# facebookresearch/habitat-lab

Hardware: AMD Instinct MI355X
Metric: env-steps/sec (SPS) PointNav RGB-D 256x256, 64 envs x 128 rollout (higher is better)
Workload: dtype f32; 1 GPU; PointNav SimpleCNN+GRU, 64 envs x 128 steps, 256x256 RGB-D synthetic; envs_per_gpu=64, rollout_steps=128, ppo_epoch=4, num_mini_batch=4, parallelism=dp1

## Files before the change

habitat-lab_amd/csrc/gemm_ops.hip:

```cpp
#include "igemm.h"
#include "igemm_dma.h"
#include "igemm_dma_wgrad.h"
#include "igemm_bf3.h"
#include "igemm_bf3_ws.h"
#include "dense_bf3.h"
#include "obs_conv_bf3.h"
#include "obs_conv_bf3_ws.h"
#include "obs_conv_patch.h"
#include "wgrad3x3_bf3.h"
#include "conv2_fwd_strip.h"
#include "conv2_dgrad_strip.h"
#include "conv3_dgrad_strip.h"
#include "obs_wgrad_bf3.h"
#include "obs_wgrad_strip.h"
#include "conv_patch_bf3.h"
#include "wgrad3x3_patch.h"
#include "prob_build.h"
#include <stdlib.h>

#include <atomic>

#include "../../include/habitat_amd.h"

namespace hab {
// ... 141 lines not shown
    if (form == HAB_CONV_DGRAD_FORM_CONV3_STRIP) HAB_TRY_FORM(conv3_dgrad_strip(d, dy, wd, mask, add, dx, stream));
    if (d.stride > 1) {
        ConvDgradMergedProb q;
        HAB_TRY(check_conv(d));
        q.g = make_geom(d);
        if (ConvDgradMergedProb::applicable(q.g)) {
            q.dy = dy; q.w = wd; q.mask = mask; q.add = add; q.dx = dx;
            q.finish();
            if (matrix_path_on(MP_RC) && q.M > 64)
                return by_width<false>(q.M, q.N, [&](auto t) { return bf3_launch<ConvDgradMergedProb, decltype(t)>(q, ws, ws_floats, 256, stream); });
            if (q.dma_ok()) return dma_launch<false>(q, ws, ws_floats, 1024, stream);
        }
    }
    for (int ph = 0; ph < d.stride; ++ph)
        for (int pw = 0; pw < d.stride; ++pw) {
            ConvDgradProb p;
            HAB_TRY(build(p, d, dy, wd, mask, add, dx, ph, pw));
            if (p.Hc <= 0 || p.Wc <= 0) continue;
            if (patch3x3_wanted(d, p.M) && p.K > 0) {
                const int rc = conv_patch_bf3_dispatch(p, patch3x3_geom(dy, p.g.Ho, p.g.Wo, d.Cout, d.H, d.W, d.pad - 2, 1), ws, ws_floats, stream);
                if (rc == HAB_OK) continue;
                if (rc != HAB_NOT_APPLICABLE) return rc;
            }
            if (p.K <= 0) {
                p.M = d.B * p.Hc * p.Wc;
                dgrad_empty_class_kernel<<<1024, 256, 0, stream>>>(p);
                HAB_LAUNCH_CHECK();
                continue;
            }
            HAB_TRY(run_igemm(p, ws, ws_floats, stream));
        }
    return HAB_OK;
}
int conv_wgrad(const ConvDesc& d, const float* x, const float* dy, float* dw_oihw, float* dbias, float* ws, size_t ws_floats,
               hipStream_t stream) {
    ConvWgradProb p;
    HAB_TRY(build(p, d, x, dy, dw_oihw, dbias));
    if (ws && matrix_path_on(MP_WGRAD_STRIP | MP_IJ_WGRAD) && wgrad3x3_bf3_shape(p))
        HAB_TRY_FORM(wgrad3x3_bf3(p, ws, ws_floats, stream));
    if (ws && !matrix_path_on(MP_IJ_WGRAD)) {
        ConvWgradProb q = p;
        q.colsum = nullptr;
        auto bias_grad = [&] { return dbias ? colsum(dy, p.N, p.K, p.N, dbias, 0, ws, ws_floats, stream) : HAB_OK; };
        if (wgrad3x3_patch_ok(p)) {
            HAB_TRY(bias_grad());
            return wgrad3x3_patch(q, ws, ws_floats, stream);
        }
        if (d.pad == 0 && p.N <= 32 && wgrad_dma_ok(q)) {
            HAB_TRY(bias_grad());
            if (rows_fit(q.M, 288, 256)) return igemm_dma_wgrad_launch<3, 3, 1>(q, ws, ws_floats, 1024, stream);
            return igemm_dma_wgrad_launch<2, 4, 1>(q, ws, ws_floats, 1024, stream);
        }
    }
    return run_igemm(p, ws, ws_floats, stream);
}
static int choose_obs_wgrad(const ObsConvWgradProb& p, const float* ws, size_t ws_floats) {
    if (!(matrix_path_on(MP_OBS) && p.quad && p.K > 4096)) return HAB_OBS_WGRAD_FORM_IGEMM;
    if (matrix_path_on(MP_OBS_PATCH | MP_OBS) && obs_wgrad_strip_covers(p, ws, ws_floats)) return HAB_OBS_WGRAD_FORM_STRIP;
    return obs_wgrad_bf3_covers(p, ws, ws_floats) ? HAB_OBS_WGRAD_FORM_IM2COL : HAB_OBS_WGRAD_FORM_IGEMM;
}
int obs_conv_wgrad(const ConvDesc& d, const ObsView& obs, const float* dy, float* dw_oihw, float* dbias, float* ws,
                   size_t ws_floats, hipStream_t stream) {
    ObsConvWgradProb p;
    HAB_TRY(build(p, d, obs, dy, dw_oihw, dbias));
    const int form = choose_obs_wgrad(p, ws, ws_floats);
    if (form == HAB_OBS_WGRAD_FORM_STRIP) HAB_TRY_FORM(obs_wgrad_strip_launch(p, ws, ws_floats, stream));
    if (form >= HAB_OBS_WGRAD_FORM_IM2COL) HAB_TRY_FORM(obs_wgrad_bf3_launch(p, ws, ws_floats, stream));
    return run_igemm(p, ws, ws_floats, stream);
}

static bool dense_wanted(long long M, long long N, long long K) {
    if (!matrix_path_on(MP_DENSE | MP_RC)) return false;
// ... 221 lines not shown
    return obs_conv_fwd(mk(B, H, W, o.C, Cout, KH, KW, stride, pad), o, w_fwd, bias, y, relu, ws, ws_floats, stream);
}
extern "C" int hab_obs_conv2d_fwd_form(const uint8_t* rgb, const float* depth, const int* rows, const float* w_fwd,
                                       const float* bias, float* y, int B, int H, int W, int Cout, int KH, int KW, int stride,
                                       int pad, int relu, const float* ws, size_t ws_floats) {
    if ((!rgb && !depth) || !w_fwd || !y) return HAB_ERR_ARG;
    ObsView o = mkobs(rgb, depth, rows, H, W);
    ObsConvFwdProb p;
    const int r = build(p, mk(B, H, W, o.C, Cout, KH, KW, stride, pad), o, w_fwd, bias, y, relu);
    if (r != HAB_OK) return r;
    return choose_obs_fwd(p, ws, ws_floats, nullptr);
}
extern "C" int hab_conv2d_dgrad(const float* dy, const float* w_dgrad, const float* relu_mask, const float* add, float* dx,
                                int B, int H, int W, int C, int Cout, int KH, int KW, int stride, int pad, float* ws,
                                size_t ws_floats, hipStream_t stream) {
    if (!dy || !w_dgrad || !dx) return HAB_ERR_ARG;
    return conv_dgrad(mk(B, H, W, C, Cout, KH, KW, stride, pad), dy, w_dgrad, relu_mask, add, dx, ws, ws_floats, stream);
}
extern "C" int hab_conv2d_dgrad_form(const float* dy, const float* w_dgrad, const float* relu_mask, const float* add, float* dx,
                                     int B, int H, int W, int C, int Cout, int KH, int KW, int stride, int pad, const float* ws,
                                     size_t ws_floats) {
    (void)ws; (void)ws_floats;
    if (!dy || !w_dgrad || !dx) return HAB_ERR_ARG;
    const ConvDesc d = mk(B, H, W, C, Cout, KH, KW, stride, pad);
    const int r = check_conv(d);
    if (r != HAB_OK) return r;
    return choose_conv_dgrad(d, dy, w_dgrad, relu_mask, add, dx);
}
extern "C" int hab_conv2d_wgrad(const float* x, const float* dy, float* dw_oihw, float* dbias, int B, int H, int W, int C, int Cout,
                                int KH, int KW, int stride, int pad, float* ws, size_t ws_floats, hipStream_t stream) {
    if (!x || !dy || !dw_oihw) return HAB_ERR_ARG;
    return conv_wgrad(mk(B, H, W, C, Cout, KH, KW, stride, pad), x, dy, dw_oihw, dbias, ws, ws_floats, stream);
}
extern "C" int hab_obs_conv2d_wgrad(const uint8_t* rgb, const float* depth, const int* rows, const float* dy, float* dw_oihw,
                                    float* dbias, int B, int H, int W, int Cout, int KH, int KW, int stride, int pad, float* ws,
                                    size_t ws_floats, hipStream_t stream) {
    if ((!rgb && !depth) || !dy || !dw_oihw) return HAB_ERR_ARG;
    ObsView o = mkobs(rgb, depth, rows, H, W);
    return obs_conv_wgrad(mk(B, H, W, o.C, Cout, KH, KW, stride, pad), o, dy, dw_oihw, dbias, ws, ws_floats, stream);
}
extern "C" int hab_obs_conv2d_wgrad_form(const uint8_t* rgb, const float* depth, const int* rows, const float* dy, float* dw_oihw,
                                         float* dbias, int B, int H, int W, int Cout, int KH, int KW, int stride, int pad, const float* ws,
                                         size_t ws_floats) {
    if ((!rgb && !depth) || !dy || !dw_oihw) return HAB_ERR_ARG;
    ObsView o = mkobs(rgb, depth, rows, H, W);
    ObsConvWgradProb p;
    const int r = build(p, mk(B, H, W, o.C, Cout, KH, KW, stride, pad), o, dy, dw_oihw, dbias);
    if (r != HAB_OK) return r;
    return choose_obs_wgrad(p, ws, ws_floats);
}
extern "C" int hab_linear_fwd(const float* x, int ldx, const float* w, int ldw, const float* bias, float* y, int ldy, int M,
                              int N, int K, int relu, int accumulate, float* ws, size_t ws_floats, hipStream_t stream) {
    return linear_fwd(x, ldx, w, ldw, bias, y, ldy, M, N, K, relu, accumulate, ws, ws_floats, stream);
}
extern "C" int hab_linear_dgrad(const float* dy, int lddy, const float* w, int ldw, const float* relu_mask, int ldmask,
                                float* dx, int lddx, int M, int n_in, int n_out, int accumulate, float* ws, size_t ws_floats,
                                hipStream_t stream) {
    return linear_dgrad(dy, lddy, w, ldw, relu_mask, ldmask, n_in, dx, lddx, M, n_in, n_out, accumulate, ws, ws_floats, stream);
}
extern "C" int hab_linear_wgrad(const float* dy, int lddy, const float* x, int ldx, float* dw, int lddw, int M, int n_out,
                                int n_in, int perm_c, int perm_hw, int accumulate, float* ws, size_t ws_floats,
                                hipStream_t stream) {
    return linear_wgrad(dy, lddy, x, ldx, dw, lddw, M, n_out, n_in, perm_c, perm_hw, accumulate, ws, ws_floats, stream);
}
extern "C" int hab_debug_dense_trace(long long* out320) {
    return (int)hipMemcpyFromSymbol(out320, HIP_SYMBOL(hab::dn_trace), sizeof(long long) * 8 * 8 * 5);
// ... 16 lines not shown
```

habitat-lab_amd/csrc/ops.h:

```cpp
#pragma once
#include "hab_common.h"

namespace hab {

struct ConvDesc {
    int B, H, W, C, Cout, KH, KW, stride, pad;
    int Creal = 0;
    int Ho() const { return (H + 2 * pad - KH) / stride + 1; }
    int Wo() const { return (W + 2 * pad - KW) / stride + 1; }
};
struct ObsView;

int conv_fwd(const ConvDesc& d, const float* x, const float* wf, const float* bias, float* y, int relu, float* ws,
             size_t ws_floats, hipStream_t stream);
int obs_conv_fwd(const ConvDesc& d, const ObsView& obs, const float* wf, const float* bias, float* y, int relu, float* ws,
                 size_t ws_floats, hipStream_t stream, const void* wimg = nullptr);
int64_t obs_conv_weight_image_floats();
int obs_conv_weight_image(const float* wf, int Cout, int KH, int KW, int C, void* img, hipStream_t stream);
int conv_dgrad(const ConvDesc& d, const float* dy, const float* wd, const float* mask, const float* add, float* dx,
               float* ws, size_t ws_floats, hipStream_t stream);
int conv_wgrad(const ConvDesc& d, const float* x, const float* dy, float* dw_oihw, float* dbias, float* ws, size_t ws_floats,
               hipStream_t stream);
int obs_conv_wgrad(const ConvDesc& d, const ObsView& obs, const float* dy, float* dw_oihw, float* dbias, float* ws,
                   size_t ws_floats, hipStream_t stream);
// ... 43 lines not shown
                  const int* frag_env, const int* frag_start, int F, int H, float* hinit, hipStream_t stream,
                  const int* env_first = nullptr);
int rnn_seq_layer_forward(int rnn_type, int H, const RnnLayerParams& lp, const RnnWork& wk, const float* x, int ldx,
                          const float* hinit, const float* cinit, const PackInfo& pk, float* ws, size_t ws_floats,
                          hipStream_t stream);
int rnn_seq_wave_forward(int rnn_type, int H, int L, const RnnLayerParams* lp, const RnnWork* wk, const float* x, int ldx,
                         const float* const* hinit, const float* const* cinit, const PackInfo& pk, float* ws, size_t ws_floats,
                         hipStream_t stream);
int rnn_seq_wave_backward(int rnn_type, int H, int L, const RnnLayerParams* lp, const float* const* w_ih_t, const RnnWork* wk, const float* x0,
                          int ldx0, const float* dout, float* dx0, int lddx0, const float* dx_mask, int ldmask, int mask_cols,
                          const PackInfo& pk, float* scratch , float* ws, size_t ws_floats, hipStream_t stream);
int rnn_step_layer_forward(int rnn_type, int H, const RnnLayerParams& lp, const float* x, int ldx, const float* h_in, int h_in_stride,
                           const float* c_in, int c_in_stride, const uint8_t* masks, int n, float* gi_scratch, float* h_out,
                           int h_out_stride, float* c_out, int c_out_stride, float* ws, size_t ws_floats, hipStream_t stream);
int rnn_seq_layer_backward(int rnn_type, int H, const RnnLayerParams& lp, const RnnWork& wk, const float* x, int ldx,
                           const float* dout, float* dx, int lddx, const float* dx_mask, int ldmask, int mask_cols,
                           const PackInfo& pk, float* scratch , float* ws, size_t ws_floats,
                           hipStream_t stream);
enum MatrixPath : int {
    MP_RC = 1 << 0,
    MP_OBS = 1 << 1,
    MP_IJ = 1 << 2,
    MP_IJ_WGRAD = 1 << 3,
    MP_PATCH3X3 = 1 << 4,
    MP_WS = 1 << 5,
    MP_OBS_PATCH = 1 << 6,
    MP_WGRAD_STRIP = 1 << 7,
    MP_CONV2_FWD = 1 << 8,
    MP_CONV2_DGRAD = 1 << 9,
    MP_DENSE = 1 << 10,
    MP_DENSE_ALL = 1 << 11,
    MP_RNN_STEPWISE = 1 << 12,
    MP_OBS_PATCH_PLAIN = 1 << 13,
    MP_DEFAULT = 2047,
};
int matrix_path_bits();
inline bool matrix_path_on(int bits) { return (matrix_path_bits() & bits) == bits; }
int rnn_tm_prepare(const uint8_t* masks, const int* rows, int B, uint8_t* frame_mask, int* iota, hipStream_t stream);
int rnn_tm_layer_forward(int rnn_type, int H, const RnnLayerParams& lp, const RnnWork& wk, const float* x, int ldx, const float* hinit,
                         const float* cinit, const uint8_t* frame_mask, int n, int T_total, int t0, int t1, float* ws, size_t ws_floats,
                         hipStream_t stream);
int rnn_tm_layer_backward(int rnn_type, int H, const RnnLayerParams& lp, const RnnWork& wk, const float* dout, float* dx, int lddx,
                          const float* dx_mask, int ldmask, int mask_cols, const uint8_t* frame_mask, const int* iota, int n, int T, int t0,
                          int t1, float* scratch, float* ws, size_t ws_floats, hipStream_t stream);
int rnn_tm_layer_param_grads(int rnn_type, int H, const RnnLayerParams& lp, const RnnWork& wk, const float* x, int ldx, int P, float* ws,
                             size_t ws_floats, hipStream_t stream);

}
```

habitat-lab_amd/csrc/wgrad3x3_bf3.h:

```cpp
#pragma once
#include "igemm_bf3.h"

namespace hab {

struct W3bArgs {
    const float* x;
    const float* dy;
    float* partial;
    int B, H, Ho;
    int strips;
    int items;
    int sign_schedule;
    int colsum;
};

template <int C32, int N32, int W, int PAD, int KHW, int S, int R, int KS, int NS>
struct W3bCfg {
    static constexpr int C = 32 * C32, N = 32 * N32, WP = W + 2 * PAD, Wo = (WP - KHW) / S + 1, NT = 64 * KHW * KS * NS, NW = N32 / NS;
    static constexpr int XRS = (R - 1) * S + KHW;
    static constexpr int XROWS = XRS * WP, NPIX = R * Wo, NQ = (NPIX + 3) / 4, NSTEPS = (NQ + 3) / 4, YROWS = NSTEPS * 16;
    static constexpr int XU = XRS * W * C / 4, YU = R * Wo * N / 4, XPT = (XU + NT - 1) / NT, YPT = (YU + NT - 1) / NT;
    static constexpr int X_HALF = XROWS * 32, Y_HALF = YROWS * 32;
    static constexpr size_t LDS_BYTES = (size_t)(3 * C32 * X_HALF + 3 * N32 * Y_HALF) * 2;
    static constexpr int WH = (WP + 1) / 2;
    __host__ __device__ static constexpr int xcol(int w) { return S == 2 ? (w & 1) * WH + (w >> 1) : w; }
    __host__ __device__ static constexpr int tap_col(int kw) { return S == 2 ? (kw & 1) * WH + (kw >> 1) : kw; }
    static_assert(S == 1 || S == 2, "");
    static_assert(LDS_BYTES % 16 == 0 && N32 % NS == 0 && NT % (N / 4) == 0 && LDS_BYTES >= (size_t)NT * 16, "");
};

typedef short w3b_v4s __attribute__((ext_vector_type(4)));
typedef short w3b_v8s __attribute__((ext_vector_type(8)));

__device__ __forceinline__ w3b_v4s w3b_tr_read(const unsigned short* p) {
    return __builtin_amdgcn_ds_read_tr16_b64_v4i16((__attribute__((address_space(3))) w3b_v4s*)p);
}
__device__ __forceinline__ bf16x8 w3b_join(const w3b_v4s lo, const w3b_v4s hi) {
    return __builtin_bit_cast(bf16x8, __builtin_shufflevector(lo, hi, 0, 1, 2, 3, 4, 5, 6, 7));
}

template <int C32, int N32, int W, int PAD, int KHW, int S, int R, int KS, int NS>
__global__ void __launch_bounds__(64 * KHW * KS * NS) wgrad3x3_bf3_kernel(const W3bArgs a) {
    using Cfg = W3bCfg<C32, N32, W, PAD, KHW, S, R, KS, NS>;
    constexpr int C = Cfg::C, N = Cfg::N, WP = Cfg::WP, Wo = Cfg::Wo, NT = Cfg::NT, NW = Cfg::NW;
    extern __shared__ __attribute__((aligned(16))) unsigned short smem16[];
    unsigned short* xs = smem16;
    unsigned short* ys = smem16 + 3 * C32 * Cfg::X_HALF;
    const int t = threadIdx.x, lane = t & 63;
    const int wave = __builtin_amdgcn_readfirstlane(t >> 6);
    const int kh = wave % KHW, ns = (wave / KHW) % NS, ks = wave / (KHW * NS);

    for (int i = t; i < (int)(Cfg::LDS_BYTES / 16); i += NT) reinterpret_cast<u32x4*>(smem16)[i] = u32x4{0u, 0u, 0u, 0u};

    const int xcd = blockIdx.x & 7, jw = blockIdx.x >> 3, wg_per_xcd = gridDim.x >> 3;
    const int per_xcd = (a.items + 7) >> 3, per_wg = (per_xcd + wg_per_xcd - 1) / wg_per_xcd;
    const int xcd_end = min(a.items, (xcd + 1) * per_xcd);
    const int first = min(xcd_end, xcd * per_xcd + jw * per_wg), last = min(xcd_end, first + per_wg);

    const bool flip = a.sign_schedule && (blockIdx.x & 1);
    const unsigned sgn2 = flip ? 0x80008000u : 0u;

// ... 109 lines not shown
        __syncthreads();
    }

    const int li = lane & 31, hi = lane >> 5;
    constexpr int MROWS = KHW * KHW * C;
    const size_t slab = (size_t)(MROWS + (a.colsum ? 1 : 0)) * N;
    float* out = a.partial + (size_t)(blockIdx.x * KS + ks) * slab;
#pragma unroll
    for (int kw = 0; kw < KHW; ++kw)
#pragma unroll
        for (int hc = 0; hc < C32; ++hc)
#pragma unroll
            for (int hn = 0; hn < NW; ++hn)
#pragma unroll
                for (int v = 0; v < 16; ++v) {
                    const int ci = (v & 3) + 8 * (v >> 2) + 4 * hi;
                    const float val = acc[kw][hc][hn][v];
                    out[(size_t)((kh * KHW + kw) * C + hc * 32 + ci) * N + (ns * NW + hn) * 32 + li] = flip ? -val : val;
                }
    if (a.colsum) {
        float* red = reinterpret_cast<float*>(smem16);
        *reinterpret_cast<f32x4*>(red + t * 4) = cs;
        __syncthreads();
        if (t < N) {
            float sum = 0.f;
            for (int q = (t >> 2); q < NT; q += N / 4) sum += red[q * 4 + (t & 3)];
            a.partial[(size_t)(blockIdx.x * KS) * slab + (size_t)MROWS * N + t] = sum;
#pragma unroll
            for (int z = 1; z < KS; ++z) a.partial[(size_t)(blockIdx.x * KS + z) * slab + (size_t)MROWS * N + t] = 0.f;
        }
    }
}

template <int C32, int N32, int W, int PAD, int KHW, int S, int R, int KS, int NS>
inline int wgrad3x3_bf3_run(const ConvWgradProb& p, float* ws, size_t ws_floats, hipStream_t stream) {
    using Cfg = W3bCfg<C32, N32, W, PAD, KHW, S, R, KS, NS>;
    const ConvGeom& g = p.g;
    W3bArgs a;
    a.x = p.x; a.dy = p.dy; a.partial = ws; a.B = g.B; a.H = g.H; a.Ho = g.Ho;
    a.strips = g.Ho / R;
    a.items = g.B * a.strips;
    a.sign_schedule = bf3_sign_schedule();
    a.colsum = p.colsum != nullptr;
    auto kern = wgrad3x3_bf3_kernel<C32, N32, W, PAD, KHW, S, R, KS, NS>;
    static const hipError_t attr_err = (Cfg::LDS_BYTES > 64 * 1024) ? hipFuncSetAttribute(reinterpret_cast<const void*>(kern), hipFuncAttributeMaxDynamicSharedMemorySize, (int)Cfg::LDS_BYTES) : hipSuccess;
    if (attr_err != hipSuccess) return (int)attr_err;
    const size_t MN = (size_t)(KHW * KHW * Cfg::C + (a.colsum ? 1 : 0)) * Cfg::N;
    const int per_cu = (int)std::min<size_t>(Cfg::NT <= 192 ? 4 : 2, (160 * 1024) / Cfg::LDS_BYTES);
    int grid = 256 * std::max(per_cu, 1);
    while (grid > 8 && (grid > a.items || (size_t)grid * KS * MN > ws_floats)) grid -= 8;
    if ((size_t)grid * KS * MN > ws_floats || (grid < 128 && a.items >= 1024)) return 1;
    kern<<<grid, Cfg::NT, Cfg::LDS_BYTES, stream>>>(a);
    HAB_LAUNCH_CHECK();
    igemm_splitk_reduce<ConvWgradProb>(p, ws, grid * KS, stream);
    HAB_LAUNCH_CHECK();
    return HAB_OK;
}

inline int wgrad3x3_bf3_shape(const ConvWgradProb& p) {
    const ConvGeom& g = p.g;
    if (p.Creal != g.C || (size_t)g.B * g.H * g.W * std::max(g.C, g.Cout) >= 0x7fffffffull / 2) return 0;
    if (g.KH == 4 && g.KW == 4 && g.stride == 2 && g.C == 32 && g.Cout == 64 && g.W == 63 && g.pad == 0 && g.Ho % 2 == 0) return 4;
    if (!(g.KH == 3 && g.KW == 3 && g.stride == 1)) return 0;
    if (g.C == 64 && g.Cout == 32 && g.W == 30 && g.pad == 0 && g.Ho % 2 == 0) return 1;
    if (g.C == 32 && g.Cout == 32 && g.W == 32 && g.pad == 1 && g.Ho % 4 == 0) return 2;
    if (g.C == 64 && g.Cout == 64 && g.W == 16 && g.pad == 1 && g.Ho % 4 == 0) return 3;
    return 0;
}
inline int wgrad3x3_bf3(const ConvWgradProb& p, float* ws, size_t ws_floats, hipStream_t stream) {
    if (!ws) return HAB_ERR_ARG;
    switch (wgrad3x3_bf3_shape(p)) {
        case 1: return wgrad3x3_bf3_run<2, 1, 30, 0, 3, 1, 2, 2, 1>(p, ws, ws_floats, stream);
        case 2: return wgrad3x3_bf3_run<1, 1, 32, 1, 3, 1, 2, 1, 1>(p, ws, ws_floats, stream);
        case 3: return wgrad3x3_bf3_run<2, 2, 16, 1, 3, 1, 4, 1, 2>(p, ws, ws_floats, stream);
        case 4: return wgrad3x3_bf3_run<1, 2, 63, 0, 4, 2, 2, 2, 1>(p, ws, ws_floats, stream);
    }
    return HAB_ERR_UNSUPPORTED;
}

}
```

habitat-lab_amd/habitat_amd/_lib.py:

```python
from __future__ import annotations

import ctypes as C
import os
from ctypes import POINTER, c_char_p, c_double, c_float, c_int, c_int32, c_int64, c_size_t, c_uint8, c_uint32, c_void_p

_HERE = os.path.dirname(os.path.abspath(__file__))
LIB_PATH = os.path.join(_HERE, "libhabitat_amd.so")

vp = c_void_p
ALLREDUCE_FN = C.CFUNCTYPE(None, c_void_p, c_int, c_float, c_void_p)
GRAD_READY_FN = C.CFUNCTYPE(None, c_int64, c_int64, c_void_p)


class HabError(RuntimeError):
    pass


class PolicyDesc(C.Structure):
    _fields_ = [(n, c_int32) for n in (
        "arch", "backbone", "baseplanes", "normalize_visual_inputs", "rnn_type", "rnn_layers", "hidden", "num_actions",
        "H", "W", "has_rgb", "has_depth", "goal_dim", "max_frames", "max_envs", "visual_order", "has_semantic",
        "num_object_categories", "has_compass", "has_gps", "action_dist", "gauss_flags")] + [("gauss_min_std", c_float),
                                                                                                ("gauss_max_std", c_float),
                                                                                                ("pointgoal_dim", c_int32),
# ... 51 lines not shown
    "hab_nav2d_rearr_vel_step": (c_int, [vp] * 15 + [c_uint32, c_uint32] + [c_int] * 9 + [c_float, c_int, c_int, vp]),
    "hab_nav2d_rearr_geo_bytes": (c_int, []),
    "hab_nav2d_rearr_geo_build": (c_int, [vp, c_size_t, vp, vp, c_int, c_int, c_int, c_int, vp]),
    "hab_nav2d_rearr_step_geo": (c_int, [vp] * 16 + [c_uint32, c_uint32] + [c_int] * 8 + [vp]),
    "hab_nav2d_rearr_vel_step_geo": (c_int, [vp] * 16 + [c_uint32, c_uint32] + [c_int] * 9 + [c_float, c_int, c_int, vp]),
    "hab_nav2d_rearr_oracle": (c_int, [vp, c_size_t] + [vp] * 6 + [c_int] * 3 + [vp]),
    "hab_nav2d_social_state_bytes": (c_int, []),
    "hab_nav2d_social_step": (c_int, [vp] * 14 + [c_uint32, c_uint32] + [c_int] * 8 + [c_float, c_int, c_float, c_int, c_int, vp]),
    "hab_obs_resize_crop": (c_int, [vp, vp, c_int, c_int, c_int, c_int, c_int, c_int, c_int, c_int, c_int, c_int, c_int, c_int, vp]),
    "hab_obs_resize_crop_form": (c_int, [vp, c_int, c_int, c_int, c_int, c_int, c_int, c_int, c_int]),
    "hab_obs_project": (c_int, [vp, c_int, vp, c_int, c_int, c_int, c_int, c_int, vp, vp, c_int, c_int, vp]),
    "hab_rollout_step_stats": (c_int, [vp, vp, vp, vp, vp, vp, vp, c_int, c_int, vp]),
    "hab_compute_returns": (c_int, [vp, vp, vp, vp, vp, c_int, c_int, c_float, c_float, c_int, c_int, vp]),
    "hab_advantages": (c_int, [vp, vp, vp, c_int, c_int, vp, vp, vp]),
    "hab_ppo_loss": (c_int, [vp, vp, vp, vp, vp, vp, vp, vp, c_int, c_float, c_float, c_float, c_int, vp, vp, vp, vp, vp]),
    "hab_ppo_loss_ver": (c_int, [vp, vp, vp, vp, vp, vp, vp, vp, c_int, c_float, c_float, c_float, c_int, vp, vp, vp, c_int64, vp, c_float,
                                 vp, vp, vp, vp, vp]),
    "hab_dagger_mix": (c_int, [vp, vp, vp, vp, vp, vp, c_float, c_float, vp, vp, vp, c_int, vp]),
    "hab_bc_loss": (c_int, [vp, vp, vp, vp, vp, vp, c_int, c_float, c_float, vp, vp, vp, vp, vp]),
    "hab_lagrange_adam_step": (c_int, [vp, vp, vp, vp, c_float, c_float, c_float, c_float, c_float, c_int, c_float, c_float, vp, vp]),
    "hab_ver_compute_returns": (c_int, [vp, vp, vp, vp, vp, vp, vp, vp, c_int, c_double, c_double, vp]),
    "hab_ver_is_coeffs": (c_int, [vp, c_int, c_int, c_int, vp, vp, vp]),
    "hab_clip_adam_step": (c_int, [vp, vp, vp, vp, c_size_t, vp, c_int, c_float, c_float, c_float, c_float, c_float,
                                   c_float, c_int, vp, vp]),
    "hab_sample_actions": (c_int, [vp, vp, vp, c_int, c_int, c_int, vp]),
    "hab_set_matrix_path": (c_int, [c_int]),
    "hab_conv2d_fwd": (c_int, [vp, vp, vp, vp] + [c_int] * 10 + [vp, c_size_t, vp]),
    "hab_obs_conv2d_fwd": (c_int, [vp, vp, vp, vp, vp, vp] + [c_int] * 9 + [vp, c_size_t, vp]),
    "hab_conv2d_dgrad": (c_int, [vp, vp, vp, vp, vp] + [c_int] * 9 + [vp, c_size_t, vp]),
    "hab_conv2d_wgrad": (c_int, [vp, vp, vp, vp] + [c_int] * 9 + [vp, c_size_t, vp]),
    "hab_obs_conv2d_wgrad": (c_int, [vp, vp, vp, vp, vp, vp] + [c_int] * 8 + [vp, c_size_t, vp]),
    "hab_obs_conv2d_wgrad_form": (c_int, [vp, vp, vp, vp, vp, vp] + [c_int] * 8 + [vp, c_size_t]),
    "hab_conv2d_dgrad_form": (c_int, [vp, vp, vp, vp, vp] + [c_int] * 9 + [vp, c_size_t]),
    "hab_obs_conv2d_fwd_form": (c_int, [vp, vp, vp, vp, vp, vp] + [c_int] * 9 + [vp, c_size_t]),
    "hab_linear_fwd": (c_int, [vp, c_int, vp, c_int, vp, vp, c_int, c_int, c_int, c_int, c_int, c_int, vp, c_size_t, vp]),
    "hab_linear_dgrad": (c_int, [vp, c_int, vp, c_int, vp, c_int, vp, c_int, c_int, c_int, c_int, c_int, vp, c_size_t, vp]),
    "hab_linear_wgrad": (c_int, [vp, c_int, vp, c_int, vp, c_int, c_int, c_int, c_int, c_int, c_int, c_int, vp, c_size_t, vp]),
    "hab_colsum": (c_int, [vp, c_int, c_int, c_int, vp, c_int, vp, c_size_t, vp]),
    "hab_repack_conv_weight": (c_int, [vp, vp, vp, c_int, c_int, c_int, c_int, c_int, vp]),
    "hab_repack_flatten_weight": (c_int, [vp, vp, c_int, c_int, c_int, vp]),
    "hab_transpose2d": (c_int, [vp, vp, c_int, c_int, vp]),
    "hab_obs_ingest_pool": (c_int, [vp, vp, vp, vp, vp, c_int, c_int, c_int, c_int, c_int, c_int, c_int, vp]),
    "hab_obs_ingest_pool_sensors": (c_int, [vp, vp, vp, vp, c_int, vp, vp, c_int, c_int, c_int, c_int, vp, vp, vp, vp, vp, vp]),
    "hab_fused_gather": (c_int, [vp, vp, c_int, vp, vp, c_int, c_int, c_int, c_int, c_int, vp]),
    "hab_channel_moments": (c_int, [vp, c_int64, c_int, c_int, vp, vp, vp, c_int, vp]),
    "hab_running_mean_var_update": (c_int, [vp, vp, vp, vp, vp, c_float, c_int, vp]),
    "hab_running_mean_var_normalize": (c_int, [vp, c_int64, c_int, c_int, vp, vp, vp]),
    "hab_groupnorm_fwd": (c_int, [vp, vp, vp, vp, vp, vp, vp, c_int, c_int, c_int, c_int, c_int, c_float, vp, c_int64, vp]),
    "hab_groupnorm_bwd": (c_int, [vp, vp, vp, vp, vp, vp, vp, vp, vp, c_int, c_int, c_int, c_int, vp, c_int64, vp]),
    "hab_split_weight_planes": (c_int, [vp, c_int, c_int, vp, vp]),
    "hab_stem_split_weights": (c_int, [vp, vp, vp]),
    "hab_stem_conv_wgrad": (c_int, [vp, vp, vp, c_int, c_int, c_int, c_int, vp, c_size_t, vp, vp]),
    "hab_stem_conv_fwd": (c_int, [vp, vp, vp, c_int, c_int, c_int, vp, vp, c_int, vp]),
    "hab_conv_gn_fwd": (c_int, [vp] * 9 + [c_int] * 11 + [c_float, vp]),
    "hab_maxpool3x3s2_fwd": (c_int, [vp, vp, vp, c_int, c_int, c_int, c_int, vp]),
    "hab_maxpool3x3s2_bwd": (c_int, [vp, vp, vp, c_int, c_int, c_int, c_int, vp]),
    "hab_nav_embed_fwd": (c_int, [POINTER(EmbedSlot), c_int, vp, vp, vp, c_int, c_int, c_int, vp, vp]),
    "hab_nav_embed_bwd": (c_int, [POINTER(EmbedSlot), c_int, vp, vp, c_int, c_int, c_int, vp, c_size_t, vp]),
    "hab_build_pack_info": (c_int, [vp, c_int, c_int] + [vp] * 12),
    "hab_build_pack_info_from_ids": (c_int, [vp, vp, vp, c_int] + [vp] * 11),
    "hab_policy_create": (c_int, [POINTER(PolicyDesc), POINTER(vp)]),
    "hab_policy_destroy": (None, [vp]),
    "hab_policy_num_params": (c_int, [vp]),
    "hab_policy_param_info": (c_int, [vp, c_int, c_char_p, c_int, POINTER(c_int64), POINTER(c_int), POINTER(c_int64)]),
    "hab_policy_param_is_buffer": (c_int, [vp, c_int]),
    "hab_policy_set_training": (c_int, [vp, c_int]),
# ... 67 lines not shown
```

include/habitat_amd.h:

```cpp
#ifndef HABITAT_AMD_H
#define HABITAT_AMD_H

#include <stddef.h>
#include <stdint.h>

#ifdef __cplusplus
extern "C" {
#endif

#ifndef __HIP_PLATFORM_AMD__
typedef struct ihipStream_t* hipStream_t;
#endif

#define HAB_ABI_VERSION 1
int hab_abi_version(void);
const char* hab_error_string(int code);

int hab_synth_step(uint8_t* rgb , float* depth , float* goal , float* reward ,
                   uint8_t* not_done , int64_t* env_t , int64_t* since_reset , uint32_t seed,
                   uint32_t env_offset, int N, int H, int W, int advance, hipStream_t stream);
int hab_synth_objectnav_sensors(int32_t* semantic, int64_t* objectgoal, float* compass, float* gps, const int64_t* env_t,
                                uint32_t seed, uint32_t env_offset, int N, int H, int W, hipStream_t stream);

#define HAB_NAV2D_STATE_BYTES 224
// ... 243 lines not shown

int hab_set_matrix_path(int mode);

int hab_conv2d_fwd(const float* x, const float* w_fwd, const float* bias, float* y, int B, int H, int W, int C, int Cout,
                   int KH, int KW, int stride, int pad, int relu, float* ws, size_t ws_floats, hipStream_t stream);
int hab_obs_conv2d_fwd(const uint8_t* rgb, const float* depth, const int* rows, const float* w_fwd, const float* bias,
                       float* y, int B, int H, int W, int Cout, int KH, int KW, int stride, int pad, int relu, float* ws,
                       size_t ws_floats, hipStream_t stream);
#define HAB_OBS_FWD_FORM_OTHER 0
#define HAB_OBS_FWD_FORM_PATCH 1
#define HAB_OBS_FWD_FORM_PATCH_PLAIN 2
int hab_obs_conv2d_fwd_form(const uint8_t* rgb, const float* depth, const int* rows, const float* w_fwd, const float* bias,
                            float* y, int B, int H, int W, int Cout, int KH, int KW, int stride, int pad, int relu, const float* ws,
                            size_t ws_floats);
int hab_conv2d_dgrad(const float* dy, const float* w_dgrad, const float* relu_mask, const float* add, float* dx, int B,
                     int H, int W, int C, int Cout, int KH, int KW, int stride, int pad, float* ws, size_t ws_floats,
                     hipStream_t stream);
int hab_conv2d_wgrad(const float* x, const float* dy, float* dw_oihw, float* dbias, int B, int H, int W, int C, int Cout,
                     int KH, int KW, int stride, int pad, float* ws, size_t ws_floats, hipStream_t stream);
int hab_obs_conv2d_wgrad(const uint8_t* rgb, const float* depth, const int* rows, const float* dy, float* dw_oihw,
                         float* dbias, int B, int H, int W, int Cout, int KH, int KW, int stride, int pad, float* ws,
                         size_t ws_floats, hipStream_t stream);
#define HAB_OBS_WGRAD_FORM_IGEMM 0
#define HAB_OBS_WGRAD_FORM_IM2COL 1
#define HAB_OBS_WGRAD_FORM_STRIP 2
int hab_obs_conv2d_wgrad_form(const uint8_t* rgb, const float* depth, const int* rows, const float* dy, float* dw_oihw,
                              float* dbias, int B, int H, int W, int Cout, int KH, int KW, int stride, int pad, const float* ws,
                              size_t ws_floats);
#define HAB_CONV_DGRAD_FORM_GENERAL 0
#define HAB_CONV_DGRAD_FORM_CONV2_STRIP 1
#define HAB_CONV_DGRAD_FORM_CONV3_STRIP 2
int hab_conv2d_dgrad_form(const float* dy, const float* w_dgrad, const float* relu_mask, const float* add, float* dx, int B,
                          int H, int W, int C, int Cout, int KH, int KW, int stride, int pad, const float* ws, size_t ws_floats);
int hab_linear_fwd(const float* x, int ldx, const float* w, int ldw, const float* bias, float* y, int ldy, int M, int N,
                   int K, int relu, int accumulate, float* ws, size_t ws_floats, hipStream_t stream);
int hab_linear_dgrad(const float* dy, int lddy, const float* w, int ldw, const float* relu_mask, int ldmask, float* dx,
                     int lddx, int M, int n_in, int n_out, int accumulate, float* ws, size_t ws_floats,
                     hipStream_t stream);
int hab_linear_wgrad(const float* dy, int lddy, const float* x, int ldx, float* dw, int lddw, int M, int n_out, int n_in,
                     int perm_c, int perm_hw, int accumulate, float* ws, size_t ws_floats, hipStream_t stream);
int hab_colsum(const float* a, int lda, int M, int N, float* out, int accumulate, float* ws, size_t ws_floats,
               hipStream_t stream);
int hab_repack_conv_weight(const float* w_oihw, float* w_fwd, float* w_dgrad, int Cout, int Cin, int KH, int KW,
                           int cin_padded, hipStream_t stream);
int hab_repack_flatten_weight(const float* w, float* w_packed, int N, int C, int HW, hipStream_t stream);
int hab_transpose2d(const float* w, float* wt, int R, int C, hipStream_t stream);

int hab_obs_ingest_pool(const uint8_t* rgb, const float* depth, const int32_t* semantic, const int* rows, float* y, int B, int H, int W,
                        int cpad, int c_rgb, int c_depth, int c_sem ,
                        hipStream_t stream);
int hab_obs_ingest_pool_sensors(const void* const* sensors, const int32_t* dtypes, const int32_t* channels, const float* scales, int n,
                                const int* rows, float* y, int B, int H, int W, int cpad, const float* norm_mean, const float* norm_var,
                                const float* pivot, double* mom_partial, int* mom_blocks, hipStream_t stream);
int hab_fused_gather(const float* const* sensors, const int32_t* widths, int n, const int* rows, float* dst, int ld, int col0, int pad0,
                     int npad, int B, hipStream_t stream);
int hab_channel_moments(const float* x, int64_t npix, int cpad, int mode, const float* mean, float* out, double* scratch,
                        int scratch_len, hipStream_t stream);
int hab_running_mean_var_update(float* r_mean, float* r_var, float* r_count, const float* b_mean, const float* b_var, float n, int C,
                                hipStream_t stream);
int hab_running_mean_var_normalize(float* x, int64_t npix, int cpad, int C, const float* mean, const float* var, hipStream_t stream);
int hab_groupnorm_fwd(const float* x, float* y, const float* gamma, const float* beta, const float* residual, float* mean,
                      float* rstd, int B, int HW, int C, int groups, int relu, float eps, float* ws, int64_t ws_floats,
                      hipStream_t stream);
int hab_groupnorm_bwd(const float* x, const float* dy, const float* relu_out, float* dx, float* dy_masked, const float* gamma,
                      const float* mean, const float* rstd, float* chan_sums, int B, int HW, int C, int groups, float* ws,
                      int64_t ws_floats, hipStream_t stream);
// ... 202 lines not shown
```

Measured before the change: 66940 env-steps/s.

## Carry overlapping input rows across strips in 3x3 conv weight-gradient kernel

Adds a carried-row variant of the bf16x3 strip weight-gradient kernel for the unpadded shapes (1 and 4). Consecutive strips of the same image reuse the overlapping input rows already in LDS, copying them down instead of refetching and re-splitting them from global memory. Shape 1 also splits the channel tiles across extra waves (HS=2) to add parallelism. A form selector and a query entry point choose between the carried and plain variants, with an env bit to force plain. The cost is more register and LDS traffic for the copy, plus a larger block size.

Result: no change. 67580 env-steps/s (median of 6 runs) (+1.0%).

```diff
diff --git a/habitat-lab_amd/csrc/gemm_ops.hip b/habitat-lab_amd/csrc/gemm_ops.hip
--- a/habitat-lab_amd/csrc/gemm_ops.hip
+++ b/habitat-lab_amd/csrc/gemm_ops.hip
@@ -197,12 +197,18 @@
         }
     return HAB_OK;
 }
+static_assert(HAB_CONV_WGRAD_FORM_OTHER == W3B_FORM_NONE && HAB_CONV_WGRAD_FORM_STRIP_CARRIED == W3B_FORM_CARRIED &&
+              HAB_CONV_WGRAD_FORM_STRIP_PLAIN == W3B_FORM_PLAIN, "");
+static int choose_conv_wgrad(const ConvWgradProb& p, const float* ws, size_t ws_floats) {
+    if (!matrix_path_on(MP_WGRAD_STRIP | MP_IJ_WGRAD)) return HAB_CONV_WGRAD_FORM_OTHER;
+    return wgrad3x3_bf3_form(p, ws, ws_floats, matrix_path_on(MP_WGRAD_STRIP_PLAIN));
+}
 int conv_wgrad(const ConvDesc& d, const float* x, const float* dy, float* dw_oihw, float* dbias, float* ws, size_t ws_floats,
                hipStream_t stream) {
     ConvWgradProb p;
     HAB_TRY(build(p, d, x, dy, dw_oihw, dbias));
-    if (ws && matrix_path_on(MP_WGRAD_STRIP | MP_IJ_WGRAD) && wgrad3x3_bf3_shape(p))
-        HAB_TRY_FORM(wgrad3x3_bf3(p, ws, ws_floats, stream));
+    const int form = choose_conv_wgrad(p, ws, ws_floats);
+    if (form != HAB_CONV_WGRAD_FORM_OTHER) HAB_TRY_FORM(wgrad3x3_bf3(p, form, ws, ws_floats, stream));
     if (ws && !matrix_path_on(MP_IJ_WGRAD)) {
         ConvWgradProb q = p;
         q.colsum = nullptr;
@@ -490,6 +496,14 @@
     if (!x || !dy || !dw_oihw) return HAB_ERR_ARG;
     return conv_wgrad(mk(B, H, W, C, Cout, KH, KW, stride, pad), x, dy, dw_oihw, dbias, ws, ws_floats, stream);
 }
+extern "C" int hab_conv2d_wgrad_form(const float* x, const float* dy, float* dw_oihw, float* dbias, int B, int H, int W, int C, int Cout,
+                                     int KH, int KW, int stride, int pad, const float* ws, size_t ws_floats) {
+    if (!x || !dy || !dw_oihw) return HAB_ERR_ARG;
+    ConvWgradProb p;
+    const int r = build(p, mk(B, H, W, C, Cout, KH, KW, stride, pad), x, dy, dw_oihw, dbias);
+    if (r != HAB_OK) return r;
+    return choose_conv_wgrad(p, ws, ws_floats);
+}
 extern "C" int hab_obs_conv2d_wgrad(const uint8_t* rgb, const float* depth, const int* rows, const float* dy, float* dw_oihw,
                                     float* dbias, int B, int H, int W, int Cout, int KH, int KW, int stride, int pad, float* ws,
                                     size_t ws_floats, hipStream_t stream) {
diff --git a/habitat-lab_amd/csrc/ops.h b/habitat-lab_amd/csrc/ops.h
--- a/habitat-lab_amd/csrc/ops.h
+++ b/habitat-lab_amd/csrc/ops.h
@@ -99,6 +99,7 @@
     MP_DENSE_ALL = 1 << 11,
     MP_RNN_STEPWISE = 1 << 12,
     MP_OBS_PATCH_PLAIN = 1 << 13,
+    MP_WGRAD_STRIP_PLAIN = 1 << 14,
     MP_DEFAULT = 2047,
 };
 int matrix_path_bits();
diff --git a/habitat-lab_amd/csrc/wgrad3x3_bf3.h b/habitat-lab_amd/csrc/wgrad3x3_bf3.h
--- a/habitat-lab_amd/csrc/wgrad3x3_bf3.h
+++ b/habitat-lab_amd/csrc/wgrad3x3_bf3.h
@@ -14,19 +14,28 @@
     int colsum;
 };
 
-template <int C32, int N32, int W, int PAD, int KHW, int S, int R, int KS, int NS>
+enum W3bForm { W3B_FORM_NONE = 0, W3B_FORM_CARRIED = 1, W3B_FORM_PLAIN = 2 };
+
+template <int C32, int N32, int W, int PAD, int KHW, int S, int R, int KS, int NS, int HS = 1, bool RING = false>
 struct W3bCfg {
-    static constexpr int C = 32 * C32, N = 32 * N32, WP = W + 2 * PAD, Wo = (WP - KHW) / S + 1, NT = 64 * KHW * KS * NS, NW = N32 / NS;
+    static constexpr int C = 32 * C32, N = 32 * N32, WP = W + 2 * PAD, Wo = (WP - KHW) / S + 1, NW = N32 / NS, CW = C32 / HS;
+    static constexpr int NTY = 64 * KHW * KS * NS, NT = NTY * HS;
     static constexpr int XRS = (R - 1) * S + KHW;
     static constexpr int XROWS = XRS * WP, NPIX = R * Wo, NQ = (NPIX + 3) / 4, NSTEPS = (NQ + 3) / 4, YROWS = NSTEPS * 16;
-    static constexpr int XU = XRS * W * C / 4, YU = R * Wo * N / 4, XPT = (XU + NT - 1) / NT, YPT = (YU + NT - 1) / NT;
+    static constexpr int XU = XRS * W * C / 4, YU = R * Wo * N / 4, YPT = (YU + NTY - 1) / NTY;
     static constexpr int X_HALF = XROWS * 32, Y_HALF = YROWS * 32;
+    static constexpr int SH = RING ? XRS - R * S : 0, XU0 = SH * W * C / 4, CROW0 = R * S;
+    static constexpr int CBLK = SH * WP * 4, CU = 3 * C32 * CBLK, CPT = (CU + NT - 1) / NT;
+    static constexpr int XPT = (XU - XU0 + NT - 1) / NT, TPT = (XU0 + NT - 1) / NT;
+    static constexpr int SPW = (NSTEPS + KS - 1) / KS;
+    static_assert(!RING || (PAD == 0 && SH > 0 && SH <= CROW0), "carried rows: unpadded, and source and destination rows apart");
+    static_assert(C32 % HS == 0, "");
     static constexpr size_t LDS_BYTES = (size_t)(3 * C32 * X_HALF + 3 * N32 * Y_HALF) * 2;
     static constexpr int WH = (WP + 1) / 2;
     __host__ __device__ static constexpr int xcol(int w) { return S == 2 ? (w & 1) * WH + (w >> 1) : w; }
     __host__ __device__ static constexpr int tap_col(int kw) { return S == 2 ? (kw & 1) * WH + (kw >> 1) : kw; }
     static_assert(S == 1 || S == 2, "");
-    static_assert(LDS_BYTES % 16 == 0 && N32 % NS == 0 && NT % (N / 4) == 0 && LDS_BYTES >= (size_t)NT * 16, "");
+    static_assert(LDS_BYTES % 16 == 0 && N32 % NS == 0 && NTY % (N / 4) == 0 && LDS_BYTES >= (size_t)NT * 16, "");
 };
 
 typedef short w3b_v4s __attribute__((ext_vector_type(4)));
@@ -202,9 +211,232 @@
     }
 }
 
+template <int C32, int N32, int W, int PAD, int KHW, int S, int R, int KS, int NS, int HS>
+__global__ void __launch_bounds__(64 * KHW * KS * NS * HS) wgrad3x3_carry_kernel(const W3bArgs a) {
+    using Cfg = W3bCfg<C32, N32, W, PAD, KHW, S, R, KS, NS, HS, true>;
+    constexpr int C = Cfg::C, N = Cfg::N, WP = Cfg::WP, Wo = Cfg::Wo, NT = Cfg::NT, NTY = Cfg::NTY, NW = Cfg::NW, CW = Cfg::CW;
+    extern __shared__ __attribute__((aligned(16))) unsigned short smem16[];
+    unsigned short* xs = smem16;
+    unsigned short* ys = smem16 + 3 * C32 * Cfg::X_HALF;
+    const int t = threadIdx.x, lane = t & 63;
+    const int wave = __builtin_amdgcn_readfirstlane(t >> 6);
+    const int kh = wave % KHW, ns = (wave / KHW) % NS, ks = (wave / (KHW * NS)) % KS, hs = wave / (KHW * NS * KS);
+
+    for (int i = t; i < (int)(Cfg::LDS_BYTES / 16); i += NT) reinterpret_cast<u32x4*>(smem16)[i] = u32x4{0u, 0u, 0u, 0u};
+
+    const int xcd = blockIdx.x & 7, jw = blockIdx.x >> 3, wg_per_xcd = gridDim.x >> 3;
+    const int per_xcd = (a.items + 7) >> 3, per_wg = (per_xcd + wg_per_xcd - 1) / wg_per_xcd;
+    const int xcd_end = min(a.items, (xcd + 1) * per_xcd);
+    const int first = min(xcd_end, xcd * per_xcd + jw * per_wg), last = min(xcd_end, first + per_wg);
+
+    const bool flip = a.sign_schedule && (blockIdx.x & 1);
+    const unsigned sgn2 = flip ? 0x80008000u : 0u;
+
+    f32x4 xr[Cfg::XPT], yr[Cfg::YPT];
+    u32x4 tc[Cfg::CPT > Cfg::TPT ? Cfg::CPT : Cfg::TPT];
+    f32x4 cs = {0.f, 0.f, 0.f, 0.f};
+    const float* pf_x = a.x;
+    bool pf_keep = false;
+    auto x_dst = [&](int u) {
+        const int c4 = u % (C / 4), pix = u / (C / 4), w = pix % W, hh = pix / W;
+        return (c4 >> 3) * Cfg::X_HALF + (hh * WP + Cfg::xcol(w)) * 32 + (c4 & 7) * 4;
+    };
+    auto c_dst = [&](int v) { return (v / Cfg::CBLK) * Cfg::X_HALF + (v % Cfg::CBLK) * 8; };
+    int xdst[Cfg::XPT], cdst[Cfg::CPT];
+#pragma unroll
+    for (int j = 0; j < Cfg::XPT; ++j) xdst[j] = x_dst(Cfg::XU0 + t + j * NT);
+#pragma unroll
+    for (int j = 0; j < Cfg::CPT; ++j) cdst[j] = c_dst(t + j * NT);
+    auto fetch = [&](int item, bool keep) {
+        const int img = item / a.strips, ho0 = (item - img * a.strips) * R;
+        pf_x = a.x + ((long long)img * a.H + ho0 * S) * (W * C);
+        pf_keep = keep;
+#pragma unroll
+        for (int j = 0; j < Cfg::XPT; ++j) {
+            const int u = Cfg::XU0 + t + j * NT;
+            xr[j] = *reinterpret_cast<const f32x4*>(pf_x + ((Cfg::XU - Cfg::XU0) % NT == 0 || u < Cfg::XU ? u * 4 : 0));
+        }
+        if (HS > 1 && t >= NTY) return;
+        const float* yb = a.dy + ((size_t)img * a.Ho + ho0) * (size_t)(Wo * N);
+#pragma unroll
+        for (int j = 0; j < Cfg::YPT; ++j) {
+            const int u = t + j * NTY;
+            const bool ok = Cfg::YU % NTY == 0 || u < Cfg::YU;
+            yr[j] = *reinterpret_cast<const f32x4*>(yb + (ok ? (size_t)u * 4 : 0));
+        }
+    };
+    auto fetch_top = [&]() {
+        if (pf_keep) {
+#pragma unroll
+            for (int j = 0; j < Cfg::CPT; ++j)
+                if (Cfg::CU % NT == 0 || t + j * NT < Cfg::CU)
+                    tc[j] = *reinterpret_cast<const u32x4*>(xs + cdst[j] + Cfg::CROW0 * WP * 32);
+        } else {
+#pragma unroll
+            for (int j = 0; j < Cfg::TPT; ++j) {
+                const int u = t + j * NT;
+                tc[j] = *reinterpret_cast<const u32x4*>(pf_x + (Cfg::XU0 % NT == 0 || u < Cfg::XU0 ? u * 4 : 0));
+            }
+        }
+    };
+    auto stage = [&]() {
+#pragma unroll
+        for (int j = 0; j < Cfg::XPT; ++j) {
+            const int u = Cfg::XU0 + t + j * NT;
+            if ((Cfg::XU - Cfg::XU0) % NT != 0 && u >= Cfg::XU) continue;
+            unsigned short* dst = xs + xdst[j];
+            bf3_store4(xr[j], dst, dst + C32 * Cfg::X_HALF, dst + 2 * C32 * Cfg::X_HALF);
+        }
+        if (pf_keep) {
+#pragma unroll
+            for (int j = 0; j < Cfg::CPT; ++j)
+                if (Cfg::CU % NT == 0 || t + j * NT < Cfg::CU)
+                    *reinterpret_cast<u32x4*>(xs + cdst[j]) = tc[j];
+        } else {
+#pragma unroll
+            for (int j = 0; j < Cfg::TPT; ++j) {
+                const int u = t + j * NT;
+                if (Cfg::XU0 % NT != 0 && u >= Cfg::XU0) continue;
+                unsigned short* dst = xs + x_dst(u);
+                bf3_store4(__builtin_bit_cast(f32x4, tc[j]), dst, dst + C32 * Cfg::X_HALF, dst + 2 * C32 * Cfg::X_HALF);
+            }
+        }
+        if (HS > 1 && t >= NTY) return;
+#pragma unroll
+        for (int j = 0; j < Cfg::YPT; ++j) {
+            const int u = t + j * NTY;
+            if (Cfg::YU % NTY != 0 && u >= Cfg::YU) continue;
+            const int c4 = u % (N / 4), pix = u / (N / 4);
+            unsigned short* dst = ys + (c4 >> 3) * Cfg::Y_HALF + pix * 32 + (c4 & 7) * 4;
+            cs += yr[j];
+            unsigned a1, a2, a3, b1, b2, b3;
+            bf3_split2(yr[j][0], yr[j][1], a1, a2, a3);
+            bf3_split2(yr[j][2], yr[j][3], b1, b2, b3);
+            *reinterpret_cast<u32x2*>(dst) = u32x2{a1 ^ sgn2, b1 ^ sgn2};
+            *reinterpret_cast<u32x2*>(dst + N32 * Cfg::Y_HALF) = u32x2{a2 ^ sgn2, b2 ^ sgn2};
+            *reinterpret_cast<u32x2*>(dst + 2 * N32 * Cfg::Y_HALF) = u32x2{a3 ^ sgn2, b3 ^ sgn2};
+        }
+    };
+
+    f32x16 acc[KHW][CW][NW];
+#pragma unroll
+    for (int kw = 0; kw < KHW; ++kw)
+#pragma unroll
+        for (int hc = 0; hc < CW; ++hc)
+#pragma unroll
+            for (int hn = 0; hn < NW; ++hn)
+#pragma unroll
+                for (int v = 0; v < 16; ++v) acc[kw][hc][hn][v] = 0.f;
+
+    const int i16 = lane & 15;
+    const int chunk_off = ((lane >> 4) & 1) * 16 + (i16 & 3) * 4;
+    const int kblk = lane >> 5;
+
+    auto frag_offsets = [&](int s, int (&yoff)[2], int (&xoff)[2]) {
+#pragma unroll
+        for (int r = 0; r < 2; ++r) {
+            const int pix = 4 * (4 * s + 2 * kblk + r) + (i16 >> 2);
+            yoff[r] = pix * 32 + chunk_off;
+            const int pc = Cfg::NPIX % 16 == 0 ? pix : (pix < Cfg::NPIX ? pix : 0);
+            const int hol = pc / Wo, wo = pc - hol * Wo;
+            xoff[r] = ((hol * S + kh) * WP + (S == 2 ? wo : wo * S)) * 32 + chunk_off;
+        }
+    };
+    auto k_step = [&](const int (&yoff)[2], const int (&xoff)[2]) {
+        bf16x8 bfr[NW][3];
+#pragma unroll
+        for (int hn = 0; hn < NW; ++hn)
+#pragma unroll
+            for (int pl = 0; pl < 3; ++pl) {
+                const unsigned short* src = ys + (pl * N32 + ns * NW + hn) * Cfg::Y_HALF;
+                bfr[hn][pl] = w3b_join(w3b_tr_read(src + yoff[0]), w3b_tr_read(src + yoff[1]));
+            }
+#pragma unroll
+        for (int kw = 0; kw < KHW; ++kw)
+#pragma unroll
+            for (int hc = 0; hc < CW; ++hc) {
+                bf16x8 afr[3];
+#pragma unroll
+                for (int pl = 0; pl < 3; ++pl) {
+                    const unsigned short* src = xs + (pl * C32 + hs * CW + hc) * Cfg::X_HALF + Cfg::tap_col(kw) * 32;
+                    afr[pl] = w3b_join(w3b_tr_read(src + xoff[0]), w3b_tr_read(src + xoff[1]));
+                }
+                constexpr int PA[6] = {2, 0, 1, 1, 0, 0}, PB[6] = {0, 2, 1, 0, 1, 0};
+#pragma unroll
+                for (int q6 = 0; q6 < 6; ++q6)
+#pragma unroll
+                    for (int hn = 0; hn < NW; ++hn)
+                        acc[kw][hc][hn] = __builtin_amdgcn_mfma_f32_32x32x16_bf16(afr[PA[q6]], bfr[hn][PB[q6]], acc[kw][hc][hn], 0, 0, 0);
+            }
+    };
+    int hy[Cfg::SPW][2], hx[Cfg::SPW][2];
+#pragma unroll
+    for (int q = 0; q < Cfg::SPW; ++q) frag_offsets(ks + q * KS, hy[q], hx[q]);
+    auto compute = [&]() {
+#pragma unroll
+        for (int q = 0; q < Cfg::SPW; ++q)
+            if (Cfg::NSTEPS % KS == 0 || ks + q * KS < Cfg::NSTEPS) k_step(hy[q], hx[q]);
+    };
+
+    __syncthreads();
+    if (first < last) {
+        fetch(first, false);
+        fetch_top();
+    }
+    for (int item = first; item < last; ++item) {
+        stage();
+        __syncthreads();
+        if (item + 1 < last) fetch(item + 1, (item + 1) % a.strips != 0);
+        compute();
+        if (item + 1 < last) fetch_top();
+        __syncthreads();
+    }
+
+    const int li = lane & 31, hi = lane >> 5;
+    constexpr int MROWS = KHW * KHW * C;
+    const size_t slab = (size_t)(MROWS + (a.colsum ? 1 : 0)) * N;
+    float* out = a.partial + (size_t)(blockIdx.x * KS + ks) * slab;
+#pragma unroll
+    for (int kw = 0; kw < KHW; ++kw)
+#pragma unroll
+        for (int hc = 0; hc < CW; ++hc)
+#pragma unroll
+            for (int hn = 0; hn < NW; ++hn)
+#pragma unroll
+                for (int v = 0; v < 16; ++v) {
+                    const int ci = (v & 3) + 8 * (v >> 2) + 4 * hi;
+                    const float val = acc[kw][hc][hn][v];
+                    out[(size_t)((kh * KHW + kw) * C + (hs * CW + hc) * 32 + ci) * N + (ns * NW + hn) * 32 + li] = flip ? -val : val;
+                }
+    if (a.colsum) {
+        float* red = reinterpret_cast<float*>(smem16);
+        if (HS == 1 || t < NTY) *reinterpret_cast<f32x4*>(red + t * 4) = cs;
+        __syncthreads();
+        if (t < N) {
+            float sum = 0.f;
+            for (int q = (t >> 2); q < NTY; q += N / 4) sum += red[q * 4 + (t & 3)];
+            a.partial[(size_t)(blockIdx.x * KS) * slab + (size_t)MROWS * N + t] = sum;
+#pragma unroll
+            for (int z = 1; z < KS; ++z) a.partial[(size_t)(blockIdx.x * KS + z) * slab + (size_t)MROWS * N + t] = 0.f;
+        }
+    }
+}
+
 template <int C32, int N32, int W, int PAD, int KHW, int S, int R, int KS, int NS>
+inline int wgrad3x3_bf3_grid(const ConvWgradProb& p, size_t ws_floats) {
+    using Cfg = W3bCfg<C32, N32, W, PAD, KHW, S, R, KS, NS>;
+    const int items = p.g.B * (p.g.Ho / R);
+    const size_t MN = (size_t)(KHW * KHW * Cfg::C + (p.colsum ? 1 : 0)) * Cfg::N;
+    const int per_cu = (int)std::min<size_t>(Cfg::NT <= 192 ? 4 : 2, (160 * 1024) / Cfg::LDS_BYTES);
+    int grid = 256 * std::max(per_cu, 1);
+    while (grid > 8 && (grid > items || (size_t)grid * KS * MN > ws_floats)) grid -= 8;
+    if ((size_t)grid * KS * MN > ws_floats || (grid < 128 && items >= 1024)) return 0;
+    return grid;
+}
+
+template <int C32, int N32, int W, int PAD, int KHW, int S, int R, int KS, int NS, bool CARRY = false, int HS = 1>
 inline int wgrad3x3_bf3_run(const ConvWgradProb& p, float* ws, size_t ws_floats, hipStream_t stream) {
-    using Cfg = W3bCfg<C32, N32, W, PAD, KHW, S, R, KS, NS>;
+    using Cfg = W3bCfg<C32, N32, W, PAD, KHW, S, R, KS, NS, HS, CARRY>;
     const ConvGeom& g = p.g;
     W3bArgs a;
     a.x = p.x; a.dy = p.dy; a.partial = ws; a.B = g.B; a.H = g.H; a.Ho = g.Ho;
@@ -212,14 +444,12 @@
     a.items = g.B * a.strips;
     a.sign_schedule = bf3_sign_schedule();
     a.colsum = p.colsum != nullptr;
-    auto kern = wgrad3x3_bf3_kernel<C32, N32, W, PAD, KHW, S, R, KS, NS>;
+    void (*kern)(const W3bArgs) = wgrad3x3_bf3_kernel<C32, N32, W, PAD, KHW, S, R, KS, NS>;
+    if constexpr (CARRY) kern = wgrad3x3_carry_kernel<C32, N32, W, PAD, KHW, S, R, KS, NS, HS>;
     static const hipError_t attr_err = (Cfg::LDS_BYTES > 64 * 1024) ? hipFuncSetAttribute(reinterpret_cast<const void*>(kern), hipFuncAttributeMaxDynamicSharedMemorySize, (int)Cfg::LDS_BYTES) : hipSuccess;
     if (attr_err != hipSuccess) return (int)attr_err;
-    const size_t MN = (size_t)(KHW * KHW * Cfg::C + (a.colsum ? 1 : 0)) * Cfg::N;
-    const int per_cu = (int)std::min<size_t>(Cfg::NT <= 192 ? 4 : 2, (160 * 1024) / Cfg::LDS_BYTES);
-    int grid = 256 * std::max(per_cu, 1);
-    while (grid > 8 && (grid > a.items || (size_t)grid * KS * MN > ws_floats)) grid -= 8;
-    if ((size_t)grid * KS * MN > ws_floats || (grid < 128 && a.items >= 1024)) return 1;
+    const int grid = wgrad3x3_bf3_grid<C32, N32, W, PAD, KHW, S, R, KS, NS>(p, ws_floats);
+    if (grid == 0) return HAB_NOT_APPLICABLE;
     kern<<<grid, Cfg::NT, Cfg::LDS_BYTES, stream>>>(a);
     HAB_LAUNCH_CHECK();
     igemm_splitk_reduce<ConvWgradProb>(p, ws, grid * KS, stream);
@@ -237,13 +467,31 @@
     if (g.C == 64 && g.Cout == 64 && g.W == 16 && g.pad == 1 && g.Ho % 4 == 0) return 3;
     return 0;
 }
-inline int wgrad3x3_bf3(const ConvWgradProb& p, float* ws, size_t ws_floats, hipStream_t stream) {
+inline int wgrad3x3_bf3_form(const ConvWgradProb& p, const float* ws, size_t ws_floats, bool plain) {
+    if (!ws) return W3B_FORM_NONE;
+    int grid = 0;
+    const int shape = wgrad3x3_bf3_shape(p);
+    switch (shape) {
+        case 1: grid = wgrad3x3_bf3_grid<2, 1, 30, 0, 3, 1, 2, 2, 1>(p, ws_floats); break;
+        case 2: grid = wgrad3x3_bf3_grid<1, 1, 32, 1, 3, 1, 2, 1, 1>(p, ws_floats); break;
+        case 3: grid = wgrad3x3_bf3_grid<2, 2, 16, 1, 3, 1, 4, 1, 2>(p, ws_floats); break;
+        case 4: grid = wgrad3x3_bf3_grid<1, 2, 63, 0, 4, 2, 2, 2, 1>(p, ws_floats); break;
+    }
+    if (grid == 0) return W3B_FORM_NONE;
+    return (shape == 1 || shape == 4) && !plain ? W3B_FORM_CARRIED : W3B_FORM_PLAIN;
+}
+inline int wgrad3x3_bf3(const ConvWgradProb& p, int form, float* ws, size_t ws_floats, hipStream_t stream) {
     if (!ws) return HAB_ERR_ARG;
+    const bool carried = form == W3B_FORM_CARRIED;
     switch (wgrad3x3_bf3_shape(p)) {
-        case 1: return wgrad3x3_bf3_run<2, 1, 30, 0, 3, 1, 2, 2, 1>(p, ws, ws_floats, stream);
+        case 1:
+            if (carried) return wgrad3x3_bf3_run<2, 1, 30, 0, 3, 1, 2, 2, 1, true, 2>(p, ws, ws_floats, stream);
+            return wgrad3x3_bf3_run<2, 1, 30, 0, 3, 1, 2, 2, 1>(p, ws, ws_floats, stream);
         case 2: return wgrad3x3_bf3_run<1, 1, 32, 1, 3, 1, 2, 1, 1>(p, ws, ws_floats, stream);
         case 3: return wgrad3x3_bf3_run<2, 2, 16, 1, 3, 1, 4, 1, 2>(p, ws, ws_floats, stream);
-        case 4: return wgrad3x3_bf3_run<1, 2, 63, 0, 4, 2, 2, 2, 1>(p, ws, ws_floats, stream);
+        case 4:
+            if (carried) return wgrad3x3_bf3_run<1, 2, 63, 0, 4, 2, 2, 2, 1, true, 1>(p, ws, ws_floats, stream);
+            return wgrad3x3_bf3_run<1, 2, 63, 0, 4, 2, 2, 2, 1>(p, ws, ws_floats, stream);
     }
     return HAB_ERR_UNSUPPORTED;
 }
diff --git a/habitat-lab_amd/habitat_amd/_lib.py b/habitat-lab_amd/habitat_amd/_lib.py
--- a/habitat-lab_amd/habitat_amd/_lib.py
+++ b/habitat-lab_amd/habitat_amd/_lib.py
@@ -107,6 +107,7 @@
     "hab_obs_conv2d_wgrad": (c_int, [vp, vp, vp, vp, vp, vp] + [c_int] * 8 + [vp, c_size_t, vp]),
     "hab_obs_conv2d_wgrad_form": (c_int, [vp, vp, vp, vp, vp, vp] + [c_int] * 8 + [vp, c_size_t]),
     "hab_conv2d_dgrad_form": (c_int, [vp, vp, vp, vp, vp] + [c_int] * 9 + [vp, c_size_t]),
+    "hab_conv2d_wgrad_form": (c_int, [vp, vp, vp, vp] + [c_int] * 9 + [vp, c_size_t]),
     "hab_obs_conv2d_fwd_form": (c_int, [vp, vp, vp, vp, vp, vp] + [c_int] * 9 + [vp, c_size_t]),
     "hab_linear_fwd": (c_int, [vp, c_int, vp, c_int, vp, vp, c_int, c_int, c_int, c_int, c_int, c_int, vp, c_size_t, vp]),
     "hab_linear_dgrad": (c_int, [vp, c_int, vp, c_int, vp, c_int, vp, c_int, c_int, c_int, c_int, c_int, vp, c_size_t, vp]),
diff --git a/include/habitat_amd.h b/include/habitat_amd.h
--- a/include/habitat_amd.h
+++ b/include/habitat_amd.h
@@ -299,6 +299,11 @@
 #define HAB_CONV_DGRAD_FORM_CONV3_STRIP 2
 int hab_conv2d_dgrad_form(const float* dy, const float* w_dgrad, const float* relu_mask, const float* add, float* dx, int B,
                           int H, int W, int C, int Cout, int KH, int KW, int stride, int pad, const float* ws, size_t ws_floats);
+#define HAB_CONV_WGRAD_FORM_OTHER 0
+#define HAB_CONV_WGRAD_FORM_STRIP_CARRIED 1
+#define HAB_CONV_WGRAD_FORM_STRIP_PLAIN 2
+int hab_conv2d_wgrad_form(const float* x, const float* dy, float* dw_oihw, float* dbias, int B, int H, int W, int C, int Cout,
+                          int KH, int KW, int stride, int pad, const float* ws, size_t ws_floats);
 int hab_linear_fwd(const float* x, int ldx, const float* w, int ldw, const float* bias, float* y, int ldy, int M, int N,
                    int K, int relu, int accumulate, float* ws, size_t ws_floats, hipStream_t stream);
 int hab_linear_dgrad(const float* dy, int lddy, const float* w, int ldw, const float* relu_mask, int ldmask, float* dx,
```
